# tum-vision/povar

Measured on AMD Instinct MI355X. Metric: power-series iterations/s (solve_pOSE terms per second), higher is better.
Workload: dtype f64

## Files before the change

povar_amd/csrc/povar_kernels_ck.hpp:

```cpp
#pragma once

#include "povar_kernels.hpp"

namespace povar {

constexpr int CK_ROWS = 16;

struct CkP {
  const double2* uv;
  const uint32_t* li;
  const double* w;
  const int4* tile;
  const int2* lane_meta;
  const int* bt_off;
  const int* slot_rec;
  int nb, slots;
  unsigned uv_bytes, li_bytes;
  const uint8_t* lcnt;
  const uint16_t* tick;
  int max_acc;
  int uv_packed;
  const int* cpos;
  double4* q4c;
  const int2* first_meta;
  const int4* first_hdr;
};
__device__ inline double ck_unpack_uv(unsigned k) {
  const double kd = (double)(int)k;
  const double q0 = kd * 1e-6;
  const double r = __builtin_fma(-q0, 1e6, kd);
  return __builtin_fma(r, 1e-6, q0);
}
typedef unsigned __attribute__((ext_vector_type(4))) ck_u4;
constexpr int CK_ACC_STRIDE = 13;
__host__ __device__ inline size_t ck_lds_bytes_dev(int slots, int n_acc, int ng) { return 16 + (size_t)ng * slots * 48 + (size_t)n_acc * CK_ACC_STRIDE * 8 + 64; }

__device__ inline void ck_barrier() { asm volatile("s_waitcnt lgkmcnt(0)\n\ts_barrier" ::: "memory"); }

__device__ inline void ck_group_barrier(int* cnt, int& gen, int group_waves, int lane) {
  asm volatile("s_waitcnt lgkmcnt(0)" ::: "memory");
  gen += group_waves;
  if (lane == 0) __hip_atomic_fetch_add(cnt, 1, __ATOMIC_RELAXED, __HIP_MEMORY_SCOPE_WORKGROUP);
  while (__hip_atomic_load(cnt, __ATOMIC_RELAXED, __HIP_MEMORY_SCOPE_WORKGROUP) < gen) __builtin_amdgcn_s_sleep(2);
  asm volatile("" ::: "memory");
}

__host__ __device__ inline int ck_rank(int x) { return x < 0 ? -1 : (x & 0xffff); }
__host__ __device__ inline int ck_seg(int x) { return ((x >> 16) & 63) | (((x >> 22) & 63) << 8); }

__device__ inline void ck_forward_math(const LplObs& o, const double* zz, const double* P3, double hx, double hy, double hz,
                                       double* red) {
  const double d0 = hx * zz[0] + hy * zz[1] + hz * zz[2] + zz[3];
  const double d1 = hx * zz[4] + hy * zz[5] + hz * zz[6] + zz[7];
  const double d2 = hx * zz[8] + hy * zz[9] + hz * zz[10] + zz[11];
  const double a0 = o.w * (d0 - o.cu * d2);
  const double a1 = o.w * (d1 - o.cv * d2);
  const double a2 = o.w * (o.cuv * d2 - o.cu * d0 - o.cv * d1);
  red[0] = P3[0] * a0 + P3[3] * a1 + P3[6] * a2;
  red[1] = P3[1] * a0 + P3[4] * a1 + P3[7] * a2;
  red[2] = P3[2] * a0 + P3[5] * a1 + P3[8] * a2;
}

__device__ inline double ck_huber_w(const Dp& d, const double* P3, double hx, double hy, double hz, double2 uv) {
  const double p0 = P3[0] * hx + P3[1] * hy + P3[2] * hz + P3[9];
  const double p1 = P3[3] * hx + P3[4] * hy + P3[5] * hz + P3[10];
  const double p2 = P3[6] * hx + P3[7] * hy + P3[8] * hz + P3[11];
  const double a = p0 - uv.x * p2, b = p1 - uv.y * p2, c = p0 - uv.x, e = p1 - uv.y;
  const double r2 = d.sb * d.sb * (a * a + b * b) + d.sa * d.sa * (c * c + e * e);
  const double t = d.huber;
  double y = __builtin_amdgcn_rsq(r2);
  const double hr = 0.5 * r2;
  y = y * __builtin_fma(-hr * y, y, 1.5);
  y = y * __builtin_fma(-hr * y, y, 1.5);
  return r2 < t * t ? 1.0 : t * y;
}

__device__ inline void ck_obs_forward(const Dp& d, double2 uv, double w, const double* zz, const double* P3, double hx, double hy,
                                      double hz, double* lu, int S, uint32_t s) {
  LplObs o;
  o.set(d, uv, w);
  double red[3];
  ck_forward_math(o, zz, P3, hx, hy, hz, red);
  __hip_atomic_fetch_add(lu + s, red[0], __ATOMIC_RELAXED, __HIP_MEMORY_SCOPE_WORKGROUP);
  __hip_atomic_fetch_add(lu + s + 1, red[1], __ATOMIC_RELAXED, __HIP_MEMORY_SCOPE_WORKGROUP);
  __hip_atomic_fetch_add(lu + s + 2, red[2], __ATOMIC_RELAXED, __HIP_MEMORY_SCOPE_WORKGROUP);
}
__device__ inline void ck_obs_backward(const Dp& d, double2 uv, double w, const double* P3, double hx, double hy, double hz,
                                       const double* g, double* y) {
  LplObs o;
  o.set(d, uv, w);
  double q[3];
  lpl_backward(o, P3, g, q);
#pragma unroll
  for (int m = 0; m < 3; ++m) {
    y[4 * m] += hx * q[m];
    y[4 * m + 1] += hy * q[m];
    y[4 * m + 2] += hz * q[m];
    y[4 * m + 3] += q[m];
  }
}

struct CkRows {
  __amdgpu_buffer_rsrc_t uv, li, w;
};
__device__ inline CkRows ck_rows(const CkP& k) {
  CkRows R;
  R.uv = __builtin_amdgcn_make_buffer_rsrc(const_cast<double2*>(k.uv), 0, k.uv_bytes, 0x00020000);
  R.li = __builtin_amdgcn_make_buffer_rsrc(const_cast<uint32_t*>(k.li), 0, k.li_bytes, 0x00020000);
  R.w = __builtin_amdgcn_make_buffer_rsrc(const_cast<double*>(k.w), 0, k.w ? (k.uv_packed ? k.uv_bytes : k.uv_bytes / 2) : 0, 0x00020000);
  return R;
}
template <int D, bool ROBUST, bool PK = false>
struct CkStream {
  double2 uv[D];
  unsigned pk[D][2];
  uint32_t w[D];
  __device__ inline void clear() {
#pragma unroll
    for (int i = 0; i < D; ++i) {
      uv[i] = make_double2(0, 0);
      pk[i][0] = pk[i][1] = 0;
      w[i] = 0xffffffffu;
    }
  }
  __device__ inline double2 get(int i) const { return PK ? make_double2(ck_unpack_uv(pk[i][0]), ck_unpack_uv(pk[i][1])) : uv[i]; }
  __device__ inline void load(const CkRows& R, int row0, int li0, int j, int h, int lane, int i) {
    j = j < 0 ? 0 : (j >= h ? h - 1 : j);
    const unsigned ul = (unsigned)lane;
    const unsigned ro = (unsigned)(row0 + j) * (unsigned)(WAVE * 16), lo = (unsigned)(li0 + (j >> 1)) * (unsigned)(WAVE * 4);
    if (PK) {
      typedef unsigned __attribute__((ext_vector_type(2))) u2;
      const u2 a = __builtin_amdgcn_raw_buffer_load_b64(R.uv, ul * 8u, ro >> 1, 0);
      pk[i][0] = a.x;
      pk[i][1] = a.y;
    } else {
      typedef unsigned __attribute__((ext_vector_type(4))) u4;
      const u4 a = __builtin_amdgcn_raw_buffer_load_b128(R.uv, ul * 16u, ro, 0);
      uv[i] = make_double2(__longlong_as_double(((long long)a.y << 32) | a.x), __longlong_as_double(((long long)a.w << 32) | a.z));
    }
    w[i] = __builtin_amdgcn_raw_buffer_load_b32(R.li, ul * 4u, lo, 0);
  }
  template <int DIR>
  __device__ inline void start(const CkRows& R, int row0, int li0, int h, int lane) {
#pragma unroll
    for (int i = 0; i < D; ++i) load(R, row0, li0, DIR > 0 ? i : h - 1 - i, h, lane, i);
  }
};
template <int D, bool ROBUST, bool PK>
__device__ inline void ck_forward_step(const Dp& d, const CkRows& k, CkStream<D, ROBUST, PK>& st, int row0, int li0, int h, int lane,
                                       const double* zz, const double* P3, const double* lh, double* lu, int S, int j, int i) {
  const double2 uv = st.get(i);
  const uint32_t s = (st.w[i] >> (16 * (j & 1))) & 0xffffu;
  st.load(k, row0, li0, j + D, h, lane, i);
  if (s != 0xffffu) {
    const double hx = lh[s], hy = lh[s + 1], hz = lh[s + 2];
    const double rw = ROBUST ? ck_huber_w(d, P3, hx, hy, hz, uv) : 1.0;
    ck_obs_forward(d, uv, rw, zz, P3, hx, hy, hz, lu, S, s);
  }
}
template <int D, bool ROBUST, bool PK>
__device__ inline void ck_forward_rows(const Dp& d, const CkRows& k, CkStream<D, ROBUST, PK>& st, int row0, int li0, int h, int lane,
                                       const double* zz, const double* P3, const double* lh, double* lu, int S) {
  int n0 = 0;
#pragma nounroll
  for (; n0 + D <= h; n0 += D) {
#pragma unroll
    for (int i = 0; i < D; ++i) ck_forward_step<D, ROBUST, PK>(d, k, st, row0, li0, h, lane, zz, P3, lh, lu, S, n0 + i, i);
  }
#pragma unroll
  for (int i = 0; i < D - 1; ++i)
    if (n0 + i < h) ck_forward_step<D, ROBUST, PK>(d, k, st, row0, li0, h, lane, zz, P3, lh, lu, S, n0 + i, i);
}
template <int D, bool ROBUST, bool PK>
__device__ inline void ck_backward_step(const Dp& d, const CkRows& k, CkStream<D, ROBUST, PK>& st, int row0, int li0, int h, int lane,
                                        const double* P3, const double* lh, const double* lg, int S, double* y, int j, int i) {
  const double2 uv = st.get(i);
  const uint32_t s = (st.w[i] >> (16 * (j & 1))) & 0xffffu;
  st.load(k, row0, li0, j - D, h, lane, i);
  if (s != 0xffffu) {
    const double hx = lh[s], hy = lh[s + 1], hz = lh[s + 2];
    const double rw = ROBUST ? ck_huber_w(d, P3, hx, hy, hz, uv) : 1.0;
    const double g[3] = {lg[s], lg[s + 1], lg[s + 2]};
    ck_obs_backward(d, uv, rw, P3, hx, hy, hz, g, y);
  }
}
template <int D, bool ROBUST, bool PK>
__device__ inline void ck_backward_rows(const Dp& d, const CkRows& k, CkStream<D, ROBUST, PK>& st, int row0, int li0, int h, int lane,
                                        const double* P3, const double* lh, const double* lg, int S, double* y) {
  int n0 = 0;
#pragma nounroll
  for (; n0 + D <= h; n0 += D) {
#pragma unroll
    for (int i = 0; i < D; ++i) ck_backward_step<D, ROBUST, PK>(d, k, st, row0, li0, h, lane, P3, lh, lg, S, y, h - 1 - (n0 + i), i);
  }
#pragma unroll
  for (int i = 0; i < D - 1; ++i)
    if (n0 + i < h) ck_backward_step<D, ROBUST, PK>(d, k, st, row0, li0, h, lane, P3, lh, lg, S, y, h - 1 - (n0 + i), i);
}

template <bool ROBUST, bool PK>
__device__ inline void ck_backward_rows_cold(const Dp& d, const CkP& k, const CkRows& R, int row0, int li0, int h, int lane,
                                             const double* P3, const double* lh, const double* lg, bool cold_lane, double* y) {
  for (int j = h - 1; j >= 0; --j) {
    CkStream<2, ROBUST, PK> one;
    one.load(R, row0, li0, j, h, lane, 0);
    const int cp = cold_lane ? k.cpos[(size_t)(row0 + j) * WAVE + lane] : -1;
    const double2 uv = one.get(0);
    const uint32_t s = (one.w[0] >> (16 * (j & 1))) & 0xffffu;
    if (s != 0xffffu) {
      const double hx = lh[s], hy = lh[s + 1], hz = lh[s + 2];
      const double rw = ROBUST ? ck_huber_w(d, P3, hx, hy, hz, uv) : 1.0;
      const double g[3] = {lg[s], lg[s + 1], lg[s + 2]};
      LplObs o;
      o.set(d, uv, rw);
      double q[3];
      lpl_backward(o, P3, g, q);
      if (cp >= 0) {
        k.q4c[cp] = make_double4(q[0], q[1], q[2], 0.0);
      } else {
#pragma unroll
        for (int m = 0; m < 3; ++m) {
          y[4 * m] += hx * q[m];
          y[4 * m + 1] += hy * q[m];
          y[4 * m + 2] += hz * q[m];
          y[4 * m + 3] += q[m];
        }
      }
    }
  }
}

__device__ inline void ck_load_z(const Dp& d, int rank, double* zz) {
  const double2* r = reinterpret_cast<const double2*>(d.hot_rec + (size_t)rank * HOT_REC_STRIDE);
#pragma unroll
  for (int j = 0; j < 6; ++j) {
    const double2 v = r[j];
    zz[2 * j] = v.x;
    zz[2 * j + 1] = v.y;
  }
}
__device__ inline __amdgpu_buffer_rsrc_t ck_zimg_rsrc(const Dp& d) {
  return __builtin_amdgcn_make_buffer_rsrc(d.zimg, 0, (unsigned)d.n_cams * 96u, 0x00020000);
}
__device__ inline void ck_load_z_img(const Dp& d, int rank, double* zz) {
  const __amdgpu_buffer_rsrc_t ZR = ck_zimg_rsrc(d);
#pragma unroll
  for (int j = 0; j < 6; ++j) {
    const ck_u4 a = __builtin_amdgcn_raw_buffer_load_b128(ZR, (unsigned)rank * 96u + 16u * j, 0, 0);
    zz[2 * j] = __hiloint2double((int)a.y, (int)a.x);
    zz[2 * j + 1] = __hiloint2double((int)a.w, (int)a.z);
  }
}
__device__ inline void ck_load_p3(const Dp& d, int rank, double* P3) {
  const double2* r = reinterpret_cast<const double2*>(d.hot_rec + (size_t)rank * HOT_REC_STRIDE) + 6;
#pragma unroll
  for (int j = 0; j < 4; ++j) {
    const double2 v = r[j];
    P3[2 * j] = v.x;
    P3[2 * j + 1] = v.y;
  }
  P3[8] = d.hot_rec[(size_t)rank * HOT_REC_STRIDE + 20];
}
template <bool ROBUST>
__device__ inline void ck_load_p(const Dp& d, int rank, double* P3) {
  ck_load_p3(d, rank, P3);
  if (ROBUST) {
    const double* r = d.hot_rec + (size_t)rank * HOT_REC_STRIDE;
    P3[9] = r[21];
    const double2 v = reinterpret_cast<const double2*>(r)[11];
    P3[10] = v.x;
    P3[11] = v.y;
  }
}

#ifndef POVAR_CK_PART_AUX
#define POVAR_CK_PART_AUX 0
#endif
__device__ inline __amdgpu_buffer_rsrc_t ck_part_rsrc(double* part_out) {
  return __builtin_amdgcn_make_buffer_rsrc(part_out, 0, 0x7ffffff0, 0x00020000);
}
__device__ inline void ck_store_part(__amdgpu_buffer_rsrc_t pr, unsigned byte_off, double a, double b) {
  ck_u4 g;
  g.x = (unsigned)__double2loint(a); g.y = (unsigned)__double2hiint(a); g.z = (unsigned)__double2loint(b); g.w = (unsigned)__double2hiint(b);
  __builtin_amdgcn_raw_buffer_store_b128(g, pr, byte_off, 0, POVAR_CK_PART_AUX);
}
__device__ inline void ck_flush_tile(double (&y)[12], int flags, int lane, int rank, int acc_slot, int seg, double* acc, int n_acc,
                                     double* part_ptr) {
  if (flags & 1) seg_scan_steps<12>(y, lane, seg & 255, 4);
  if (rank >= 0) {
    if (acc_slot >= 0) {
      if (lane == ((seg >> 8) & 255)) {
#pragma unroll
        for (int m = 0; m < 12; ++m)
          __hip_atomic_fetch_add(acc + acc_slot * CK_ACC_STRIDE + m, y[m], __ATOMIC_RELAXED, __HIP_MEMORY_SCOPE_WORKGROUP);
      }
    } else if (part_ptr) {
      const __amdgpu_buffer_rsrc_t part_out = ck_part_rsrc(part_ptr);
      const unsigned o = (unsigned)(~acc_slot) * 96u;
#pragma unroll
      for (int m = 0; m < 6; ++m) ck_store_part(part_out, o + 16u * m, y[2 * m], y[2 * m + 1]);
    }
  }
}

template <int NW, int SD, bool DB, int NG, bool ROBUST, bool PK>
__global__ __launch_bounds__(NW * 64) void e0_ck(Dp d, CkP k, double* part_out) {
  const int done = d.flags[1];
  extern __shared__ double ck_lds[];
  constexpr int GW = NW / NG;
  const CkRows R = ck_rows(k);
  const int S = k.slots;
  const int lane0 = threadIdx.x & 63;
  const int wave_all = __builtin_amdgcn_readfirstlane((int)(threadIdx.x >> 6));
  const int grp = NG > 1 ? wave_all / GW : 0;
  const int wave = NG > 1 ? wave_all % GW : wave_all;
  int* gbase = reinterpret_cast<int*>(ck_lds);
  double* lh = ck_lds + 2 + (size_t)grp * 6 * S;
  double* lu = lh + 3 * S;
  double* acc = ck_lds + 2 + (size_t)NG * 6 * S;
  int* gcnt = gbase + grp;
  int ggen = 0;
  const V2& v = d.v2;
  const int cam0 = v.wg_cam_off[blockIdx.x];
  const int n_acc = v.wg_cam_off[blockIdx.x + 1] - cam0;
  const int t0 = __builtin_amdgcn_readfirstlane(v.wg_tile_off[blockIdx.x]);
  const int t1 = __builtin_amdgcn_readfirstlane(v.wg_tile_off[blockIdx.x + 1]);
  typedef const int __attribute__((address_space(4))) * cint_p;
  const cint_p tiles = (cint_p)(uintptr_t)k.tile;
  const cint_p bt = (cint_p)(uintptr_t)k.bt_off;
  if (done) return;
  auto group_barrier = [&]() {
    if (NG > 1) ck_group_barrier(gcnt, ggen, GW, lane0);
    else ck_barrier();
  };
  const int wave_t = (wave & ~3) | (((wave >> 2) & 1) ? 3 - (wave & 3) : (wave & 3));
  auto tile_of = [&](int tb0, int q) { return tb0 + q * GW + ((q & 1) ? GW - 1 - wave_t : wave_t); };
  constexpr int HM = 32 / NW > 0 ? 32 / NW : 1;
  double hn[HM][3];
  auto request_h = [&](int b, int lane) {
#pragma unroll
    for (int q = 0; q < HM; ++q) {
      hn[q][0] = hn[q][1] = hn[q][2] = 0;
      const int m = wave + q * GW;
      if (b < k.nb && t0 + b + k.nb * m < t1) {
        const double* rp = v.lmrec + ((size_t)(t0 + b + k.nb * m) * 9) * WAVE + lane;
        hn[q][0] = rp[0]; hn[q][1] = rp[WAVE]; hn[q][2] = rp[2 * WAVE];
      }
    }
  };
  int* lbt = reinterpret_cast<int*>(acc + (size_t)k.max_acc * CK_ACC_STRIDE);
  const bool bt_lds = k.nb + 1 <= 16;
  auto bt_of = [&](int i, bool first) {
    return (bt_lds && !first) ? __builtin_amdgcn_readfirstlane(lbt[i]) : bt[blockIdx.x * k.nb + i];
  };
  constexpr bool EARLY = !ROBUST && SD == 2;
  int tb0_next = 0, tb1_next = 0, rank_next = 0, rank_next2 = 0;
  ck_u4 hdr_next = {0, 0, 0, 0};
  auto request_first_meta = [&](int b, int lane, bool ranks) {
    tb0_next = tb1_next = 0;
    if (b < k.nb) {
      tb0_next = bt_of(b, b == grp);
      tb1_next = bt_of(b + 1, b == grp);
// ... 67 lines not shown
  for (int b = grp; b < k.nb; b += NG) {
    int lane = lane0;
    asm volatile("" : "+v"(lane));
    const int tb0 = tb0_next, tb1 = tb1_next;
    int q_t = 0;
    int t = tile_of(tb0, 0);
    int rank = rank_next;
    int tn = tile_of(tb0, 1);
    if (!EARLY) request_first_tile(lane, t < tb1);
    int rank_n = rank_next2, rank_nn = 0;
    double zn[12] = {0, 0, 0, 0, 0, 0, 0, 0, 0, 0, 0, 0}, Pn[12] = {0, 0, 0, 0, 0, 0, 0, 0, 0, 0, 0, 0};
    CkStream<SD, ROBUST, PK> stn;
    stn.clear();
    int row0n = 0, hnx = 0, fln = 0, li0n = 0;
#pragma unroll
    for (int q = 0; q < HM; ++q) {
      const int m = wave + q * GW;
      if (t0 + b + k.nb * m < t1) {
        const int s = m * WAVE + lane;
        lh[3 * s] = hn[q][0];
        lh[3 * s + 1] = hn[q][1];
        lh[3 * s + 2] = hn[q][2];
        lu[3 * s] = 0;
        lu[3 * s + 1] = 0;
        lu[3 * s + 2] = 0;
      }
    }
    for (int m = wave + HM * GW; t0 + b + k.nb * m < t1; m += GW) {
      const double* rp = v.lmrec + ((size_t)(t0 + b + k.nb * m) * 9) * WAVE + lane;
      const int s = m * WAVE + lane;
      lh[3 * s] = rp[0];
      lh[3 * s + 1] = rp[WAVE];
      lh[3 * s + 2] = rp[2 * WAVE];
      lu[3 * s] = 0;
      lu[3 * s + 1] = 0;
      lu[3 * s + 2] = 0;
    }
    auto request_next_fwd = [&]() {
      if (DB && tn < tb1) {
        const int tnn = tile_of(tb0, q_t + 2);
        row0n = tiles[4 * tn]; hnx = tiles[4 * tn + 1]; fln = tiles[4 * tn + 2]; li0n = tiles[4 * tn + 3];
        if (tnn < tb1) rank_nn = ck_rank(k.lane_meta[(size_t)tnn * WAVE + lane].x);
        const int rk = rank_n < 0 ? 0 : rank_n;
        ck_load_z_img(d, rk, zn);
        ck_load_p<ROBUST>(d, rk, Pn);
        stn.template start<1>(R, row0n, li0n, hnx, lane);
      }
    };
    request_next_fwd();
    group_barrier();
#pragma unroll
    for (int e = 0; e < 12; ++e) asm volatile("" : "+v"(zz[e]));
    while (t < tb1) {
      ck_forward_rows<SD, ROBUST, PK>(d, R, st, row0, li0, h, lane, zz, P3, lh, lu, S);
      if (tn >= tb1) break;
      t = tn;
      ++q_t;
      rank = rank_n;
      tn = tile_of(tb0, q_t + 1);
      if (DB) {
#pragma unroll
        for (int e = 0; e < 12; ++e) zz[e] = zn[e];
#pragma unroll
        for (int e = 0; e < (ROBUST ? 12 : 9); ++e) P3[e] = Pn[e];
        st = stn;
        row0 = row0n; h = hnx; fl = fln; li0 = li0n;
        rank_n = rank_nn;
        request_next_fwd();
      } else {
        row0 = tiles[4 * t]; h = tiles[4 * t + 1]; fl = tiles[4 * t + 2]; li0 = tiles[4 * t + 3];
        if (tn < tb1) rank_n = ck_rank(k.lane_meta[(size_t)tn * WAVE + lane].x);
        const int rk = rank < 0 ? 0 : rank;
        ck_load_z_img(d, rk, zz);
        ck_load_p<ROBUST>(d, rk, P3);
        st.template start<1>(R, row0, li0, h, lane);
      }
    }
    asm volatile("" : "+v"(lane));
    int acc_slot = 0, seg = 0;
    int tp = q_t > 0 ? tile_of(tb0, q_t - 1) : tb1;
    int rank_p = 0, acc_p = 0, seg_p = 0, rank_pp = 0, acc_pp = 0, seg_pp = 0;
    double G[HM][6];
#pragma unroll
    for (int q = 0; q < HM; ++q) {
#pragma unroll
      for (int e = 0; e < 6; ++e) G[q][e] = 0;
      const int m = wave + q * GW;
      if (t0 + b + k.nb * m < t1) {
        const double* rp = v.lmrec + ((size_t)(t0 + b + k.nb * m) * 9 + 3) * WAVE + lane;
#pragma unroll
        for (int e = 0; e < 6; ++e) G[q][e] = rp[e * WAVE];
      }
    }
    if (t < tb1) {
      const int2 me = k.lane_meta[(size_t)t * WAVE + lane];
      seg = ck_seg(me.x);
      acc_slot = me.y;
      if (tp < tb1) {
        const int2 mp = k.lane_meta[(size_t)tp * WAVE + lane];
        rank_p = ck_rank(mp.x);
        seg_p = ck_seg(mp.x);
        acc_p = mp.y;
      }
      st.template start<-1>(R, row0, li0, h, lane);
    }
    group_barrier();
    request_first_meta(b + NG, lane, true);
    request_h(b + NG, lane);
#pragma unroll
    for (int q = 0; q < HM; ++q) {
      const int m = wave + q * GW;
      if (t0 + b + k.nb * m < t1) {
        const int s = m * WAVE + lane;
        const double u0 = lu[3 * s], u1 = lu[3 * s + 1], u2 = lu[3 * s + 2];
        lu[3 * s] = G[q][0] * u0 + G[q][1] * u1 + G[q][2] * u2;
        lu[3 * s + 1] = G[q][1] * u0 + G[q][3] * u1 + G[q][4] * u2;
        lu[3 * s + 2] = G[q][2] * u0 + G[q][4] * u1 + G[q][5] * u2;
      }
    }
    for (int m = wave + HM * GW; t0 + b + k.nb * m < t1; m += GW) {
      const double* rp = v.lmrec + ((size_t)(t0 + b + k.nb * m) * 9 + 3) * WAVE + lane;
      const double g0 = rp[0], g1 = rp[WAVE], g2 = rp[2 * WAVE], g3 = rp[3 * WAVE], g4 = rp[4 * WAVE], g5 = rp[5 * WAVE];
      const int s = m * WAVE + lane;
      const double u0 = lu[3 * s], u1 = lu[3 * s + 1], u2 = lu[3 * s + 2];
      lu[3 * s] = g0 * u0 + g1 * u1 + g2 * u2;
      lu[3 * s + 1] = g1 * u0 + g3 * u1 + g4 * u2;
      lu[3 * s + 2] = g2 * u0 + g4 * u1 + g5 * u2;
    }
    auto request_next_bwd = [&]() {
      if (DB && tp < tb1) {
        const int tpp = q_t > 1 ? tile_of(tb0, q_t - 2) : tb1;
        row0n = tiles[4 * tp]; hnx = tiles[4 * tp + 1]; fln = tiles[4 * tp + 2]; li0n = tiles[4 * tp + 3];
        if (tpp < tb1) {
          const int2 mp = k.lane_meta[(size_t)tpp * WAVE + lane];
          rank_pp = ck_rank(mp.x);
          seg_pp = ck_seg(mp.x);
          acc_pp = mp.y;
        }
        ck_load_p<ROBUST>(d, rank_p < 0 ? 0 : rank_p, Pn);
        stn.template start<-1>(R, row0n, li0n, hnx, lane);
      }
    };
    request_next_bwd();
    group_barrier();
    while (t < tb1) {
      double y[12];
#pragma unroll
      for (int m = 0; m < 12; ++m) y[m] = 0;
      const bool cold_q = !ROBUST && k.cpos != nullptr && (fl & 2) != 0;
      if (cold_q) ck_backward_rows_cold<ROBUST, PK>(d, k, R, row0, li0, h, lane, P3, lh, lu, rank >= 0 && acc_slot < 0, y);
      else ck_backward_rows<SD, ROBUST, PK>(d, R, st, row0, li0, h, lane, P3, lh, lu, S, y);
      ck_flush_tile(y, fl, lane, rank, acc_slot, seg, acc, n_acc, cold_q ? nullptr : part_out);
      if (tp >= tb1) break;
      t = tp;
      --q_t;
      rank = rank_p; acc_slot = acc_p; seg = seg_p;
      tp = q_t > 0 ? tile_of(tb0, q_t - 1) : tb1;
      if (DB) {
#pragma unroll
        for (int e = 0; e < (ROBUST ? 12 : 9); ++e) P3[e] = Pn[e];
        st = stn;
        row0 = row0n; h = hnx; fl = fln; li0 = li0n;
        rank_p = rank_pp; acc_p = acc_pp; seg_p = seg_pp;
        request_next_bwd();
      } else {
        row0 = tiles[4 * t]; h = tiles[4 * t + 1]; fl = tiles[4 * t + 2]; li0 = tiles[4 * t + 3];
        if (tp < tb1) {
          const int2 mp = k.lane_meta[(size_t)tp * WAVE + lane];
          rank_p = ck_rank(mp.x);
          seg_p = ck_seg(mp.x);
          acc_p = mp.y;
        }
        ck_load_p<ROBUST>(d, rank < 0 ? 0 : rank, P3);
        st.template start<-1>(R, row0, li0, h, lane);
      }
    }
    if (EARLY) request_first_tile(lane, tile_of(tb0_next, 0) < tb1_next);
    group_barrier();
  }
  if (NG > 1) ck_barrier();
  const __amdgpu_buffer_rsrc_t PR = ck_part_rsrc(part_out);
  for (int i = threadIdx.x; i < n_acc * 6; i += NW * 64) {
    const int r = i / 6, m = 2 * (i % 6);
    const int rec = k.slot_rec[cam0 + r];
    ck_store_part(PR, (unsigned)rec * 96u + 16u * (unsigned)(i % 6), acc[r * CK_ACC_STRIDE + m], acc[r * CK_ACC_STRIDE + m + 1]);
  }
  if (d.p2p_epoch && blockIdx.x == 0 && threadIdx.x == 0) *d.p2p_epoch += 1;
}

POVAR_KERNEL __launch_bounds__(256) void ck_gather_w(const int* src, const double* w_lpl, double* w_ck, int64_t n) {
  const int64_t i = (int64_t)blockIdx.x * 256 + threadIdx.x;
  if (i >= n) return;
  const int s = src[i];
  w_ck[i] = s >= 0 ? w_lpl[s] : 0.0;
}

}
```

povar_amd/csrc/povar_kernels_ck_det.hpp:

```cpp
#pragma once

#include "povar_kernels_ck.hpp"
#include "povar_kernels_ck_joint.hpp"

namespace povar {

constexpr int CK_FIX_BITS = 61;
__device__ inline int ck_xp(double v) { return v > 0.0 ? __builtin_amdgcn_frexp_exp(v) : (v == 0.0 ? INT_MIN : 0); }
__device__ inline unsigned long long ck_fix(double x, int e) {
  const double xs = __builtin_ldexp(x, e) + 0.5;
  const double hi = __builtin_floor(xs * 0x1p-32);
  const double lo = __builtin_fma(hi, -0x1p32, xs);
  const int ih = (int)hi;
  const unsigned il = (unsigned)lo;
  return ((unsigned long long)(unsigned)ih << 32) | il;
}
__device__ inline double ck_unfix(unsigned long long v, int e) {
  const int ih = (int)(unsigned)(v >> 32);
  const unsigned il = (unsigned)v;
  return __builtin_ldexp(__builtin_fma((double)ih, 0x1p32, (double)il), -e);
}
__host__ __device__ inline size_t ck_lds_bytes_det(int slots, int n_acc) {
  return ck_lds_bytes_dev(slots, n_acc, 1) + 2 * ((size_t)slots + n_acc) + 16;
}
// ... 92 lines not shown
    ck_barrier();
#pragma unroll
    for (int pass = 0; pass < 2; ++pass) {
      for (int q = 0;; ++q) {
        const int t = tile_of(tb0, q);
        if (t >= tb1) break;
        const int row0 = tiles[4 * t], h = tiles[4 * t + 1], li0 = tiles[4 * t + 3];
        if (q > 0 || (pass > 0 && !one_tile)) {
          const int rank = ck_rank(k.lane_meta[(size_t)t * WAVE + lane].x), rk = rank < 0 ? 0 : rank;
          ck_load_z(d, rk, zz);
          ck_load_p<ROBUST>(d, rk, P3);
        }
        if (q > 0 || pass > 0) st.template start<1>(R, row0, li0, h, lane);
        if (pass == 0) ckd_forward_rows<SD, ROBUST, 0>(d, R, st, row0, li0, h, lane, zz, P3, lh, lu, lexp);
        else ckd_forward_rows<SD, ROBUST, 1>(d, R, st, row0, li0, h, lane, zz, P3, lh, lu, lexp);
      }
      if (pass == 0) {
        ck_barrier();
        for (int m = wave; t0 + b + k.nb * m < t1; m += NW) {
          const int s = m * WAVE + lane;
          const int e = (int)(unsigned)__double_as_longlong(lu[3 * s]);
          const int lc = k.lcnt[(size_t)(t0 + b + k.nb * m) * WAVE + lane];
          lexp[s] = (short)((e == INT_MIN || lc == 255) ? 0 : CK_FIX_BITS - (e + lc));
          lu[3 * s] = 0;
        }
      }
      ck_barrier();
    }
    for (int m = wave; t0 + b + k.nb * m < t1; m += NW) {
      const double* rp = v.lmrec + ((size_t)(t0 + b + k.nb * m) * 9 + 3) * WAVE + lane;
      const double g0 = rp[0], g1 = rp[WAVE], g2 = rp[2 * WAVE], g3 = rp[3 * WAVE], g4 = rp[4 * WAVE], g5 = rp[5 * WAVE];
      const int s = m * WAVE + lane;
      const int e = lexp[s];
      const double u0 = ck_unfix(__double_as_longlong(lu[3 * s]), e), u1 = ck_unfix(__double_as_longlong(lu[3 * s + 1]), e),
                   u2 = ck_unfix(__double_as_longlong(lu[3 * s + 2]), e);
      lu[3 * s] = g0 * u0 + g1 * u1 + g2 * u2;
      lu[3 * s + 1] = g1 * u0 + g3 * u1 + g4 * u2;
      lu[3 * s + 2] = g2 * u0 + g4 * u1 + g5 * u2;
    }
    asm volatile("" : "+v"(lane));
    ck_barrier();
    for (int q = 0;; ++q) {
      const int t = tile_of(tb0, q);
      if (t >= tb1) break;
      const int row0 = tiles[4 * t], h = tiles[4 * t + 1], fl = tiles[4 * t + 2], li0 = tiles[4 * t + 3];
      const int2 me = k.lane_meta[(size_t)t * WAVE + lane];
      const int rank = ck_rank(me.x), seg = ck_seg(me.x), acc_slot = me.y;
      const int my_ticket = k.tick[(size_t)t * WAVE + lane];
      if (q > 0 || !one_tile) ck_load_p<ROBUST>(d, rank < 0 ? 0 : rank, P3);
      st.template start<-1>(R, row0, li0, h, lane);
      double y[12];
#pragma unroll
      for (int m = 0; m < 12; ++m) y[m] = 0;
      ck_backward_rows<SD, ROBUST>(d, R, st, row0, li0, h, lane, P3, lh, lu, S, y);
      if (fl & 1) seg_scan_steps<12>(y, lane, seg & 255, 4);
      bool pending = false;
      if (rank >= 0) {
        if (acc_slot >= 0) {
          pending = lane == ((seg >> 8) & 255);
        } else {
          double2* o = reinterpret_cast<double2*>(part_out + (size_t)(~acc_slot) * 12);
#pragma unroll
          for (int m = 0; m < 6; ++m) o[m] = make_double2(y[2 * m], y[2 * m + 1]);
        }
      }
      const int a_slot = pending ? acc_slot : 0;
      int spins = 0;
      while (__builtin_amdgcn_ballot_w64(pending) != 0) {
        const bool give_up = ++spins > (1 << 20);
        if (pending && (give_up || __hip_atomic_load(tick + a_slot, __ATOMIC_ACQUIRE, __HIP_MEMORY_SCOPE_WORKGROUP) == (short)my_ticket)) {
          double* a = acc + a_slot * CK_ACC_STRIDE;
#pragma unroll
          for (int m = 0; m < 12; ++m) a[m] += y[m];
          __hip_atomic_store(tick + a_slot, (short)(my_ticket + 1), __ATOMIC_RELEASE, __HIP_MEMORY_SCOPE_WORKGROUP);
          if (give_up) atomicOr(&d.flags[0], 8);
          pending = false;
        } else if (pending) {
          __builtin_amdgcn_s_sleep(1);
        }
      }
    }
    ck_barrier();
  }
  for (int i = threadIdx.x; i < n_acc * 6; i += NW * 64) {
    const int r = i / 6, m = 2 * (i % 6);
    const int rec = k.slot_rec[cam0 + r];
    reinterpret_cast<double2*>(part_out + (size_t)rec * 12)[i % 6] = make_double2(acc[r * CK_ACC_STRIDE + m], acc[r * CK_ACC_STRIDE + m + 1]);
  }
}

__host__ __device__ inline size_t ckh_lds_bytes_det(int n_acc) { return ckh_lds_bytes(n_acc) + 2 * ((size_t)CKH_STRIDE + n_acc) + 16; }

template <int D, bool ROBUST, int PASS>
__device__ inline void ckhd_forward_rows(const CkRows& R, CkStreamH<D, ROBUST>& st, int row0, int li0, int h, int lane,
                                         const Cam& P, const double4 (&zz)[3], const double* lx, double* lu, const short* lexp) {
  auto step = [&](int j, int i) {
    const uint32_t s = (st.w[i] >> (16 * (j & 1))) & 0xffffu;
    const double rw = ROBUST ? st.rw[i] : 1.0;
    st.load(R, row0, li0, j + D, h, lane, i);
    if (s != 0xffffu) {
      const double4 X = make_double4(lx[s], lx[CKH_STRIDE + s], lx[2 * CKH_STRIDE + s], lx[3 * CKH_STRIDE + s]);
      const double sw = ROBUST ? sqrt(rw) : 1.0;
      const Hom hp = ckh_project(P, X);
      double t[2];
      hom_jp_x(hp, X, sw, zz, t);
      const double e0 = sw * hp.D00 * t[0], e1 = sw * hp.D00 * t[1], e2 = sw * (hp.D02 * t[0] + hp.D12 * t[1]);
      const double v[4] = {P.r0.x * e0 + P.r1.x * e1 + P.r2.x * e2, P.r0.y * e0 + P.r1.y * e1 + P.r2.y * e2,
// ... 166 lines not shown
```

povar_amd/csrc/povar_series.hip:

```cpp
#include "povar_ctx.hpp"

static CkP ck_params(const povar_ctx* c, const povar_ctx::CkDev& D) {
  return CkP{D.packed ? reinterpret_cast<const double2*>(D.uvp.p) : D.uv.p, D.li.p, D.w.p, D.tile.p, D.lane_meta.p, D.bt_off.p, D.slot_rec.p,
             D.nb, D.slots, (unsigned)(D.src.n * (D.packed ? sizeof(int2) : sizeof(double2))), (unsigned)(D.li.n * sizeof(uint32_t)),
             D.lcnt.p, D.tick.p, D.max_acc, D.packed ? 1 : 0, D.cold_q ? D.cpos.p : nullptr, c->q4c.p,
             D.first_meta.p, D.first_hdr.p};
}

static bool ck_variant_fits(const povar_ctx* c, int variant) {
  const CkVariant v = ck_variant_info(variant);
  return c->ck.ready && c->ck.nb % v.ng == 0 && ck_lds_bytes(c->ck.slots, c->ck.max_acc, v.ng) <= (size_t)CK_LDS_BYTES;
}

TermPlan term_plan(const povar_ctx* c, int step, TermUse use, int variant) {
  TermPlan p;
  p.step = step;
  p.use = use;
  const int mode = c->opt.e0_mode;
  const bool lpl = lpl_mode(c);
  const bool series = use == TermUse::series || use == TermUse::series_norms;
  if (step == 1) {
    if (variant < 0) variant = c->ck_variant;
    const povar_ctx::CkDev& D = c->ck;
    if (c->fp32_terms && use != TermUse::dense) {
// ... 139 lines not shown
    c->ev_kind.push_back(-1);
  }
  c->ev_kind[c->ev_used] = kind;
  (void)hipEventRecord(c->ev[c->ev_used], c->stream);
  ++c->ev_used;
}

Dp ldsacc_dp(povar_ctx* c, bool long_in_kernel) {
  Dp dt = c->d;
  dt.cmv = CmView{c->cc_slot.p, c->cc_h.p, c->n_cold, c->cc_item_off.p, c->cc_cam_item_off.p, c->cc_part.p,
                  c->n_cold_items, c->cc_cam_range.p};
  dt.hot_part = c->hot_part.p;
  dt.q4c = c->q4c.p;
  dt.cold_pos = c->cold_pos.p;
  if (lpl_mode(c)) {
    dt.cmv.h = c->c3_h.p;
    dt.cmv.n = c->n_cold3;
    dt.cmv.cam_range = c->c3_range.p;
    dt.cmv.src = c->q_rows ? c->c3_src.p : nullptr;
    dt.q_rows = c->q_rows ? 1 : 0;
    dt.hot_part = c->v2_part.p;
    dt.part_range = c->v2_part_range.p;
    dt.cold_pos = nullptr;
    dt.long_in_kernel = 1;
    return dt;
  }
  if (long_in_kernel && c->long_in_kernel) {
    dt.cmv.h = c->c2_h.p;
    dt.cmv.n = c->n_cold2;
    dt.cmv.cam_range = c->c2_range.p;
    dt.cold_pos = c->c2_pos.p;
    dt.long_in_kernel = 1;
  }
  return dt;
}


static Dp term_dp(povar_ctx* c, const TermPlan& p) {
  if (p.cam == CamStep::scatter || p.cam == CamStep::scatter_sum) return c->d;
  Dp d = ldsacc_dp(c, p.e0 != E0K::tiles_cached);
  if (p.ck()) {
    ck_dp(c, p.step, d);
    if (p.step == 1) d.long_in_kernel = 1;
  }
  if (p.exch == Exch::p2p) p2p_dp(c, d);
  return d;
}

template <int NW, int SD, bool DB, int NG>
void launch_e0_ck_t(povar_ctx* c, const Dp& da) {
  const CkP k = ck_params(c, c->ck);
  const size_t lds = ck_lds_bytes(c->ck.slots, c->ck.max_acc, NG);
  const bool huber = c->opt.robust_norm == POVAR_NORM_HUBER;
  if (c->ck.packed) {
    if (huber) hipLaunchKernelGGL((e0_ck<NW, SD, DB, NG, true, true>), dim3(c->e0c_grid), dim3(NW * 64), lds, c->stream, da, k, c->ck.part.p);
    else hipLaunchKernelGGL((e0_ck<NW, SD, DB, NG, false, true>), dim3(c->e0c_grid), dim3(NW * 64), lds, c->stream, da, k, c->ck.part.p);
  } else {
    if (huber) hipLaunchKernelGGL((e0_ck<NW, SD, DB, NG, true, false>), dim3(c->e0c_grid), dim3(NW * 64), lds, c->stream, da, k, c->ck.part.p);
    else hipLaunchKernelGGL((e0_ck<NW, SD, DB, NG, false, false>), dim3(c->e0c_grid), dim3(NW * 64), lds, c->stream, da, k, c->ck.part.p);
  }
}

void launch_ck32_records(povar_ctx* c) {
  const int64_t n_rec = (int64_t)c->d.v2.n_tiles * 9 * WAVE;
  const int64_t n = std::max<int64_t>(n_rec, (int64_t)c->n_cams * 12);
  hipLaunchKernelGGL(ck32_records, dim3(grid_for(n, 256)), dim3(256), 0, c->stream, (const double*)c->v2_lmrec.p, c->ck32_lmrec.p,
                     n_rec, (const double*)c->hot_rec.p, c->ck32_pimg.p, c->n_cams);
}

static void ensure_ck_w(povar_ctx* c, int step) {
  povar_ctx::CkDev& D = step == 2 ? c->ckh : c->ck;
  if (!c->opt.robust_norm || !D.ready || !D.w.p || !c->v2_w.p || D.w_lin_id == c->lin_id) return;
  const int64_t n = (int64_t)D.src.n;
  hipLaunchKernelGGL(ck_gather_w, dim3(grid_for(n, 256)), dim3(256), 0, c->stream, (const int*)D.src.p, (const double*)c->v2_w.p,
                     D.w.p, n);
  D.w_lin_id = c->lin_id;
}

int launch_e0(povar_ctx* c, const TermPlan& p) {
  if (p.use != TermUse::timing) prof_mark(c, 0);
  if (!lpl_mode(c)) ensure_legacy(c);
  if (p.ck()) ensure_ck_w(c, p.step);
  const Dp da = term_dp(c, p);
  const bool robust = c->opt.robust_norm != 0, huber = c->opt.robust_norm == POVAR_NORM_HUBER;
  const dim3 grid(c->e0c_grid);
  switch (p.e0) {
    case E0K::ck_f32: {
      const CkP k = ck_params(c, c->ck);
      const Ck32 f{c->ck.packed ? nullptr : c->ck32_uv.p, c->ck32_lmrec.p, c->ck32_pimg.p,
                   (unsigned)(c->ck.src.n * sizeof(float2)), (unsigned)(c->ck.part.n * sizeof(double))};
      const size_t lds = ck32_lds_bytes(c->ck.slots, c->ck.max_acc);
      const dim3 block(CK32_NW * 64);
      if (c->ck.packed) {
        if (huber) hipLaunchKernelGGL((e0_ck_f32<true, true>), grid, block, lds, c->stream, da, k, f, c->ck.part.p);
        else hipLaunchKernelGGL((e0_ck_f32<false, true>), grid, block, lds, c->stream, da, k, f, c->ck.part.p);
      } else {
        if (huber) hipLaunchKernelGGL((e0_ck_f32<true, false>), grid, block, lds, c->stream, da, k, f, c->ck.part.p);
        else hipLaunchKernelGGL((e0_ck_f32<false, false>), grid, block, lds, c->stream, da, k, f, c->ck.part.p);
      }
      break;
    }
    case E0K::ck_det: {
      const size_t lds = ck_lds_bytes_det(c->ck.slots, c->ck.max_acc);
      if (huber) hipLaunchKernelGGL((e0_ck_det<16, 2, true>), grid, dim3(1024), lds, c->stream, da, ck_params(c, c->ck), c->ck.part.p);
      else hipLaunchKernelGGL((e0_ck_det<16, 2, false>), grid, dim3(1024), lds, c->stream, da, ck_params(c, c->ck), c->ck.part.p);
      break;
    }
    case E0K::ck:
      switch (p.variant) {
#define X(id, nw, sd, db, ng) case id: launch_e0_ck_t<nw, sd, db, ng>(c, da); break;
        POVAR_CK_VARIANTS(X)
#undef X
// ... 608 lines not shown
```

Measured before the change: 19280.

## Fold per-row projection constants into P3 and z for non-robust e0_ck path

For the non-robust case the kernel now precomputes row constants (rho, scales, kappa) on the host and pre-scales P3 and the third z row once per tile. The per-observation forward and backward work then reduces to a short FMA formula instead of the general LplObs setup and lpl_backward. The aim is to cut per-observation ALU work in the hot power-series loop. The identity depends on kappa being fixed at 1 and on correct rescaling of y and q4c, so numerical equivalence needs checking.

```diff
diff --git a/povar_amd/csrc/povar_kernels_ck.hpp b/povar_amd/csrc/povar_kernels_ck.hpp
--- a/povar_amd/csrc/povar_kernels_ck.hpp
+++ b/povar_amd/csrc/povar_kernels_ck.hpp
@@ -6,6 +6,18 @@
 
 constexpr int CK_ROWS = 16;
 
+struct CkRowK {
+  double rho;
+  double s01;
+  double s2;
+  double kz;
+  double yf;
+};
+__host__ inline CkRowK ck_row_consts(double sa, double sb) {
+  const double kappa = 1.0, sb2 = sb * sb;
+  if (sb2 == 0.0) return CkRowK{0.0, 1.0, 0.0, 0.0, 0.0};
+  return CkRowK{(sa * sa) / sb2, sb2, -kappa * sb2, kappa, -kappa};
+}
 struct CkP {
   const double2* uv;
   const uint32_t* li;
@@ -100,6 +112,46 @@
   }
 }
 
+__device__ inline void ck_scale_p3(const CkRowK& c, double* P3) {
+#pragma unroll
+  for (int e = 0; e < 6; ++e) P3[e] *= c.s01;
+#pragma unroll
+  for (int e = 6; e < 9; ++e) P3[e] *= c.s2;
+}
+template <int SGN>
+__device__ inline void ck_apply_c_m(double rho, double2 kp, double x0, double x1, double x2, double* a) {
+  const double m0 = __builtin_fma(SGN > 0 ? -kp.x : kp.x, x2, x0), m1 = __builtin_fma(SGN > 0 ? -kp.y : kp.y, x2, x1);
+  a[0] = __builtin_fma(rho, x0, m0);
+  a[1] = __builtin_fma(rho, x1, m1);
+  a[2] = __builtin_fma(kp.y, m1, kp.x * m0);
+}
+__device__ inline void ck_obs_forward_m(double rho, double2 kp, const double* zz, const double* P3, double hx, double hy, double hz,
+                                        double* lu, uint32_t s) {
+  const double d0 = __builtin_fma(hx, zz[0], __builtin_fma(hy, zz[1], __builtin_fma(hz, zz[2], zz[3])));
+  const double d1 = __builtin_fma(hx, zz[4], __builtin_fma(hy, zz[5], __builtin_fma(hz, zz[6], zz[7])));
+  const double d2 = __builtin_fma(hx, zz[8], __builtin_fma(hy, zz[9], __builtin_fma(hz, zz[10], zz[11])));
+  double a[3];
+  ck_apply_c_m<1>(rho, kp, d0, d1, d2, a);
+  __hip_atomic_fetch_add(lu + s, P3[0] * a[0] + P3[3] * a[1] + P3[6] * a[2], __ATOMIC_RELAXED, __HIP_MEMORY_SCOPE_WORKGROUP);
+  __hip_atomic_fetch_add(lu + s + 1, P3[1] * a[0] + P3[4] * a[1] + P3[7] * a[2], __ATOMIC_RELAXED, __HIP_MEMORY_SCOPE_WORKGROUP);
+  __hip_atomic_fetch_add(lu + s + 2, P3[2] * a[0] + P3[5] * a[1] + P3[8] * a[2], __ATOMIC_RELAXED, __HIP_MEMORY_SCOPE_WORKGROUP);
+}
+__device__ inline void ck_q_m(double rho, double2 kp, const double* P3, const double* g, double* q) {
+  const double e0 = P3[0] * g[0] + P3[1] * g[1] + P3[2] * g[2];
+  const double e1 = P3[3] * g[0] + P3[4] * g[1] + P3[5] * g[2];
+  const double f = P3[6] * g[0] + P3[7] * g[1] + P3[8] * g[2];
+  ck_apply_c_m<-1>(rho, kp, e0, e1, f, q);
+}
+__device__ inline void ck_add_outer(double hx, double hy, double hz, const double* q, double* y) {
+#pragma unroll
+  for (int m = 0; m < 3; ++m) {
+    y[4 * m] += hx * q[m];
+    y[4 * m + 1] += hy * q[m];
+    y[4 * m + 2] += hz * q[m];
+    y[4 * m + 3] += q[m];
+  }
+}
+
 struct CkRows {
   __amdgpu_buffer_rsrc_t uv, li, w;
 };
@@ -146,60 +198,72 @@
     for (int i = 0; i < D; ++i) load(R, row0, li0, DIR > 0 ? i : h - 1 - i, h, lane, i);
   }
 };
-template <int D, bool ROBUST, bool PK>
-__device__ inline void ck_forward_step(const Dp& d, const CkRows& k, CkStream<D, ROBUST, PK>& st, int row0, int li0, int h, int lane,
-                                       const double* zz, const double* P3, const double* lh, double* lu, int S, int j, int i) {
+template <int D, bool ROBUST, bool PK, bool MF = false>
+__device__ inline void ck_forward_step(const Dp& d, double rho, const CkRows& k, CkStream<D, ROBUST, PK>& st, int row0, int li0, int h,
+                                       int lane, const double* zz, const double* P3, const double* lh, double* lu, int S, int j, int i) {
   const double2 uv = st.get(i);
   const uint32_t s = (st.w[i] >> (16 * (j & 1))) & 0xffffu;
   st.load(k, row0, li0, j + D, h, lane, i);
   if (s != 0xffffu) {
     const double hx = lh[s], hy = lh[s + 1], hz = lh[s + 2];
-    const double rw = ROBUST ? ck_huber_w(d, P3, hx, hy, hz, uv) : 1.0;
-    ck_obs_forward(d, uv, rw, zz, P3, hx, hy, hz, lu, S, s);
-  }
-}
-template <int D, bool ROBUST, bool PK>
-__device__ inline void ck_forward_rows(const Dp& d, const CkRows& k, CkStream<D, ROBUST, PK>& st, int row0, int li0, int h, int lane,
-                                       const double* zz, const double* P3, const double* lh, double* lu, int S) {
+    if (!MF) {
+      const double rw = ROBUST ? ck_huber_w(d, P3, hx, hy, hz, uv) : 1.0;
+      ck_obs_forward(d, uv, rw, zz, P3, hx, hy, hz, lu, S, s);
+    } else {
+      ck_obs_forward_m(rho, uv, zz, P3, hx, hy, hz, lu, s);
+    }
+  }
+}
+template <int D, bool ROBUST, bool PK, bool MF = false>
+__device__ inline void ck_forward_rows(const Dp& d, double rho, const CkRows& k, CkStream<D, ROBUST, PK>& st, int row0, int li0, int h,
+                                       int lane, const double* zz, const double* P3, const double* lh, double* lu, int S) {
   int n0 = 0;
 #pragma nounroll
   for (; n0 + D <= h; n0 += D) {
 #pragma unroll
-    for (int i = 0; i < D; ++i) ck_forward_step<D, ROBUST, PK>(d, k, st, row0, li0, h, lane, zz, P3, lh, lu, S, n0 + i, i);
+    for (int i = 0; i < D; ++i) ck_forward_step<D, ROBUST, PK, MF>(d, rho, k, st, row0, li0, h, lane, zz, P3, lh, lu, S, n0 + i, i);
   }
 #pragma unroll
   for (int i = 0; i < D - 1; ++i)
-    if (n0 + i < h) ck_forward_step<D, ROBUST, PK>(d, k, st, row0, li0, h, lane, zz, P3, lh, lu, S, n0 + i, i);
-}
-template <int D, bool ROBUST, bool PK>
-__device__ inline void ck_backward_step(const Dp& d, const CkRows& k, CkStream<D, ROBUST, PK>& st, int row0, int li0, int h, int lane,
-                                        const double* P3, const double* lh, const double* lg, int S, double* y, int j, int i) {
+    if (n0 + i < h) ck_forward_step<D, ROBUST, PK, MF>(d, rho, k, st, row0, li0, h, lane, zz, P3, lh, lu, S, n0 + i, i);
+}
+template <int D, bool ROBUST, bool PK, bool MF = false>
+__device__ inline void ck_backward_step(const Dp& d, double rho, const CkRows& k, CkStream<D, ROBUST, PK>& st, int row0, int li0, int h,
+                                        int lane, const double* P3, const double* lh, const double* lg, int S, double* y, int j, int i) {
   const double2 uv = st.get(i);
   const uint32_t s = (st.w[i] >> (16 * (j & 1))) & 0xffffu;
   st.load(k, row0, li0, j - D, h, lane, i);
   if (s != 0xffffu) {
     const double hx = lh[s], hy = lh[s + 1], hz = lh[s + 2];
-    const double rw = ROBUST ? ck_huber_w(d, P3, hx, hy, hz, uv) : 1.0;
-    const double g[3] = {lg[s], lg[s + 1], lg[s + 2]};
-    ck_obs_backward(d, uv, rw, P3, hx, hy, hz, g, y);
-  }
-}
-template <int D, bool ROBUST, bool PK>
-__device__ inline void ck_backward_rows(const Dp& d, const CkRows& k, CkStream<D, ROBUST, PK>& st, int row0, int li0, int h, int lane,
-                                        const double* P3, const double* lh, const double* lg, int S, double* y) {
+    if (!MF) {
+      const double rw = ROBUST ? ck_huber_w(d, P3, hx, hy, hz, uv) : 1.0;
+      const double g[3] = {lg[s], lg[s + 1], lg[s + 2]};
+      ck_obs_backward(d, uv, rw, P3, hx, hy, hz, g, y);
+    } else {
+      const double g[3] = {lg[s], lg[s + 1], lg[s + 2]};
+      double q[3];
+      ck_q_m(rho, uv, P3, g, q);
+      ck_add_outer(hx, hy, hz, q, y);
+    }
+  }
+}
+template <int D, bool ROBUST, bool PK, bool MF = false>
+__device__ inline void ck_backward_rows(const Dp& d, double rho, const CkRows& k, CkStream<D, ROBUST, PK>& st, int row0, int li0, int h,
+                                        int lane, const double* P3, const double* lh, const double* lg, int S, double* y) {
   int n0 = 0;
 #pragma nounroll
   for (; n0 + D <= h; n0 += D) {
 #pragma unroll
-    for (int i = 0; i < D; ++i) ck_backward_step<D, ROBUST, PK>(d, k, st, row0, li0, h, lane, P3, lh, lg, S, y, h - 1 - (n0 + i), i);
+    for (int i = 0; i < D; ++i)
+      ck_backward_step<D, ROBUST, PK, MF>(d, rho, k, st, row0, li0, h, lane, P3, lh, lg, S, y, h - 1 - (n0 + i), i);
   }
 #pragma unroll
   for (int i = 0; i < D - 1; ++i)
-    if (n0 + i < h) ck_backward_step<D, ROBUST, PK>(d, k, st, row0, li0, h, lane, P3, lh, lg, S, y, h - 1 - (n0 + i), i);
-}
-
-template <bool ROBUST, bool PK>
-__device__ inline void ck_backward_rows_cold(const Dp& d, const CkP& k, const CkRows& R, int row0, int li0, int h, int lane,
+    if (n0 + i < h) ck_backward_step<D, ROBUST, PK, MF>(d, rho, k, st, row0, li0, h, lane, P3, lh, lg, S, y, h - 1 - (n0 + i), i);
+}
+
+template <bool ROBUST, bool PK, bool MF>
+__device__ inline void ck_backward_rows_cold(const Dp& d, const CkRowK& rk, const CkP& k, const CkRows& R, int row0, int li0, int h, int lane,
                                              const double* P3, const double* lh, const double* lg, bool cold_lane, double* y) {
   for (int j = h - 1; j >= 0; --j) {
     CkStream<2, ROBUST, PK> one;
@@ -209,22 +273,20 @@
     const uint32_t s = (one.w[0] >> (16 * (j & 1))) & 0xffffu;
     if (s != 0xffffu) {
       const double hx = lh[s], hy = lh[s + 1], hz = lh[s + 2];
-      const double rw = ROBUST ? ck_huber_w(d, P3, hx, hy, hz, uv) : 1.0;
       const double g[3] = {lg[s], lg[s + 1], lg[s + 2]};
-      LplObs o;
-      o.set(d, uv, rw);
       double q[3];
-      lpl_backward(o, P3, g, q);
+      if (!MF) {
+        const double rw = ROBUST ? ck_huber_w(d, P3, hx, hy, hz, uv) : 1.0;
+        LplObs o;
+        o.set(d, uv, rw);
+        lpl_backward(o, P3, g, q);
+      } else {
+        ck_q_m(rk.rho, uv, P3, g, q);
+      }
       if (cp >= 0) {
-        k.q4c[cp] = make_double4(q[0], q[1], q[2], 0.0);
+        k.q4c[cp] = make_double4(q[0], q[1], MF ? rk.yf * q[2] : q[2], 0.0);
       } else {
-#pragma unroll
-        for (int m = 0; m < 3; ++m) {
-          y[4 * m] += hx * q[m];
-          y[4 * m + 1] += hy * q[m];
-          y[4 * m + 2] += hz * q[m];
-          y[4 * m + 3] += q[m];
-        }
+        ck_add_outer(hx, hy, hz, q, y);
       }
     }
   }
@@ -304,10 +366,11 @@
 }
 
 template <int NW, int SD, bool DB, int NG, bool ROBUST, bool PK>
-__global__ __launch_bounds__(NW * 64) void e0_ck(Dp d, CkP k, double* part_out) {
+__global__ __launch_bounds__(NW * 64) void e0_ck(Dp d, CkP k, double* part_out, CkRowK rk) {
   const int done = d.flags[1];
   extern __shared__ double ck_lds[];
   constexpr int GW = NW / NG;
+  constexpr bool MF = !ROBUST;
   const CkRows R = ck_rows(k);
   const int S = k.slots;
   const int lane0 = threadIdx.x & 63;
@@ -481,7 +544,12 @@
 #pragma unroll
     for (int e = 0; e < 12; ++e) asm volatile("" : "+v"(zz[e]));
     while (t < tb1) {
-      ck_forward_rows<SD, ROBUST, PK>(d, R, st, row0, li0, h, lane, zz, P3, lh, lu, S);
+      if (MF) {
+        ck_scale_p3(rk, P3);
+#pragma unroll
+        for (int e = 8; e < 12; ++e) zz[e] *= rk.kz;
+      }
+      ck_forward_rows<SD, ROBUST, PK, MF>(d, rk.rho, R, st, row0, li0, h, lane, zz, P3, lh, lu, S);
       if (tn >= tb1) break;
       t = tn;
       ++q_t;
@@ -572,13 +640,20 @@
     };
     request_next_bwd();
     group_barrier();
+    bool p3_fresh = false;
     while (t < tb1) {
       double y[12];
 #pragma unroll
       for (int m = 0; m < 12; ++m) y[m] = 0;
+      if (MF && p3_fresh) ck_scale_p3(rk, P3);
+      p3_fresh = true;
       const bool cold_q = !ROBUST && k.cpos != nullptr && (fl & 2) != 0;
-      if (cold_q) ck_backward_rows_cold<ROBUST, PK>(d, k, R, row0, li0, h, lane, P3, lh, lu, rank >= 0 && acc_slot < 0, y);
-      else ck_backward_rows<SD, ROBUST, PK>(d, R, st, row0, li0, h, lane, P3, lh, lu, S, y);
+      if (cold_q) ck_backward_rows_cold<ROBUST, PK, MF>(d, rk, k, R, row0, li0, h, lane, P3, lh, lu, rank >= 0 && acc_slot < 0, y);
+      else ck_backward_rows<SD, ROBUST, PK, MF>(d, rk.rho, R, st, row0, li0, h, lane, P3, lh, lu, S, y);
+      if (MF) {
+#pragma unroll
+        for (int m = 8; m < 12; ++m) y[m] *= rk.yf;
+      }
       ck_flush_tile(y, fl, lane, rank, acc_slot, seg, acc, n_acc, cold_q ? nullptr : part_out);
       if (tp >= tb1) break;
       t = tp;
diff --git a/povar_amd/csrc/povar_kernels_ck_det.hpp b/povar_amd/csrc/povar_kernels_ck_det.hpp
--- a/povar_amd/csrc/povar_kernels_ck_det.hpp
+++ b/povar_amd/csrc/povar_kernels_ck_det.hpp
@@ -168,7 +168,7 @@
       double y[12];
 #pragma unroll
       for (int m = 0; m < 12; ++m) y[m] = 0;
-      ck_backward_rows<SD, ROBUST>(d, R, st, row0, li0, h, lane, P3, lh, lu, S, y);
+      ck_backward_rows<SD, ROBUST, false>(d, 0.0, R, st, row0, li0, h, lane, P3, lh, lu, S, y);
       if (fl & 1) seg_scan_steps<12>(y, lane, seg & 255, 4);
       bool pending = false;
       if (rank >= 0) {
diff --git a/povar_amd/csrc/povar_series.hip b/povar_amd/csrc/povar_series.hip
--- a/povar_amd/csrc/povar_series.hip
+++ b/povar_amd/csrc/povar_series.hip
@@ -215,12 +215,13 @@
   const CkP k = ck_params(c, c->ck);
   const size_t lds = ck_lds_bytes(c->ck.slots, c->ck.max_acc, NG);
   const bool huber = c->opt.robust_norm == POVAR_NORM_HUBER;
+  const CkRowK rk = ck_row_consts(da.sa, da.sb);
   if (c->ck.packed) {
-    if (huber) hipLaunchKernelGGL((e0_ck<NW, SD, DB, NG, true, true>), dim3(c->e0c_grid), dim3(NW * 64), lds, c->stream, da, k, c->ck.part.p);
-    else hipLaunchKernelGGL((e0_ck<NW, SD, DB, NG, false, true>), dim3(c->e0c_grid), dim3(NW * 64), lds, c->stream, da, k, c->ck.part.p);
+    if (huber) hipLaunchKernelGGL((e0_ck<NW, SD, DB, NG, true, true>), dim3(c->e0c_grid), dim3(NW * 64), lds, c->stream, da, k, c->ck.part.p, rk);
+    else hipLaunchKernelGGL((e0_ck<NW, SD, DB, NG, false, true>), dim3(c->e0c_grid), dim3(NW * 64), lds, c->stream, da, k, c->ck.part.p, rk);
   } else {
-    if (huber) hipLaunchKernelGGL((e0_ck<NW, SD, DB, NG, true, false>), dim3(c->e0c_grid), dim3(NW * 64), lds, c->stream, da, k, c->ck.part.p);
-    else hipLaunchKernelGGL((e0_ck<NW, SD, DB, NG, false, false>), dim3(c->e0c_grid), dim3(NW * 64), lds, c->stream, da, k, c->ck.part.p);
+    if (huber) hipLaunchKernelGGL((e0_ck<NW, SD, DB, NG, true, false>), dim3(c->e0c_grid), dim3(NW * 64), lds, c->stream, da, k, c->ck.part.p, rk);
+    else hipLaunchKernelGGL((e0_ck<NW, SD, DB, NG, false, false>), dim3(c->e0c_grid), dim3(NW * 64), lds, c->stream, da, k, c->ck.part.p, rk);
   }
 }
 
```

Result: no change. 19360 (median of 6 runs) (+0.4%).
